# dafyddstephenson/ucla-roms

Hardware: AMD Instinct MI355X
Metric: grid-cell-updates/sec (higher is better)
Workload: dtype f64; 1 GPU; C3: basin 1024x1024x100, NONLIN+SPLIT EOS, T+S, LMD KPP/BKPP/RIMIX/NONLOCAL, dt=300s, ndtfast=60 (nfast=82); NT=2, nfast=82, parallelism=domain decomposition 1x1, halo_transport=none (single rank), fast_exchange_interval=1, exchange_order=none (single rank), s2d_window=True, comm_bootstrap=none (single rank)

## Files before the change

### include/roms_gpu.h

```cpp
#ifndef ROMS_GPU_H
#define ROMS_GPU_H

#ifdef __cplusplus
extern "C" {
#endif

#define ROMS_GPU_ABI_VERSION 18
#define ROMS_MAX_FAST 288

typedef struct roms_dims {
  int Lm, Mm, N, NT;
  int LLm, MMm;
  int np_xi, np_eta, inode, jnode;
  int iSW_corn, jSW_corn;
  int ew_periodic, ns_periodic;
  int west_exchng, east_exchng, south_exchng, north_exchng;
} roms_dims;

#define ROMS_LMD_MIXING   1
#define ROMS_LMD_KPP      2
#define ROMS_LMD_BKPP     4
#define ROMS_LMD_RIMIX    8
#define ROMS_LMD_CONVEC   16
#define ROMS_LMD_NONLOCAL 32
#define ROMS_LMD_ALL      63
#define ROMS_LMD_ICELAND  47
#define ROMS_LMD_DDMIX    64

typedef struct roms_cfg {
  int nonlin_eos;
  int salinity;
  int lmd_mixing;
  int uv_vis2, ts_dif2;
  double dt;
  int ndtfast, nfast;
  double weight[2][ROMS_MAX_FAST];
  double g, rho0, rdrg, rdrg2, Zob, gamma2;
  double Akv_bak, Akt_bak[2];
  double Tcoef, T0, Scoef, S0;
  double theta_s, theta_b, hc;
// ... 76 lines not shown

enum roms_case_id { ROMS_CASE_FILAMENT = 0, ROMS_CASE_BASIN = 1, ROMS_CASE_PIPES = 2, ROMS_CASE_RIVERS = 3 };
typedef struct roms_case {
  int case_id, LLm, MMm, N, NT;
  int salinity, nonlin_eos, lmd_mixing;
  double dt; int ndtfast;
  double sizex, sizey;
  int surf_flux;
  int obc;
  double v_sponge;
  int island;
  int curvgrid;
  int uv_adv, uv_cor;
  int bulk_frc;
  int adv_isoneutral;
} roms_case;
int roms_gpu_init_case(const roms_case *c, int device, roms_tlev *t);
int roms_gpu_init_case_comm(const roms_case *c, int np_xi, int np_eta, void *comm, int device, roms_tlev *t);

int roms_gpu_comm_unique_id(void *id128);
int roms_gpu_comm_create(const void *id128, int nranks, int rank, int device, void **comm);
int roms_gpu_comm_create_local(int group, int nranks, int rank, void **comm);
typedef int (*roms_host_allgather_fn)(void *ctx, const void *send, long nbytes, void *recv);
int roms_gpu_comm_create_host(int nranks, int rank, int device, roms_host_allgather_fn allgather, void *ctx,
                              void **comm);
int roms_gpu_comm_destroy(void *comm);
int roms_gpu_halo_transport(void);
int roms_gpu_halo_exchanges(long *per_step, int *fast_interval);
int roms_gpu_halo_overlap(void);
int roms_gpu_s2d_window(void);
#define ROMS_COLPATH_SEG 1
#define ROMS_COLPATH_GLOBAL 2
int roms_gpu_column_path(void);
int roms_gpu_horizontal_path(int out[8]);
int roms_gpu_selftest_zero_fill(long n, int chunks, long *bad);
int roms_gpu_halo_plan(int Lm, int Mm, int np_xi, int np_eta, int inode, int jnode, int ew_periodic,
                       int ns_periodic, int peer[8], long count[8], int strip[4]);
long roms_gpu_halo_map(int Lm, int Mm, int np_xi, int np_eta, int inode, int jnode, int ew_periodic,
                       int ns_periodic, int dir, int unpack, int *i, int *j, long cap);
long roms_gpu_halo_map_wide(int Lm, int Mm, int np_xi, int np_eta, int inode, int jnode, int ew_periodic,
                            int ns_periodic, int width, int dir, int unpack, int *i, int *j, long cap);

#define ROMS_FRC_SURFACE 1
#define ROMS_FRC_BRY     2
int roms_gpu_frc_record(int field_id, int slot, double rec_time, const double *data);
int roms_gpu_frc_interp(double modtime, int kinds);
int roms_gpu_frc_clock(double start_time, int on);
int roms_gpu_set_tide_data(int ntides, const double *ftide, const double *pot_re, const double *pot_im,
                           const double *ztide_re, const double *ztide_im, const double *utide_re,
                           const double *utide_im, const double *vtide_re, const double *vtide_im);
int roms_gpu_set_tides(double time);

#define ROMS_WRT_Z    1
#define ROMS_WRT_UB   2
#define ROMS_WRT_VB   4
#define ROMS_WRT_U    8
#define ROMS_WRT_V    16
#define ROMS_WRT_T    32
#define ROMS_WRT_R    64
#define ROMS_WRT_O    128
#define ROMS_WRT_AKV  256
#define ROMS_WRT_AKT  512
#define ROMS_WRT_AKS  1024
#define ROMS_WRT_HBLS 2048
#define ROMS_WRT_HBBL 4096
#define ROMS_WRT_DEFAULT 63
// ... 30 lines not shown
```

### ucla-roms_amd/csrc/k_lmd.hip

```cpp
#include <cmath>
#include <type_traits>

#include "k_common.h"

namespace roms {
namespace {

constexpr double kRicr = 0.15, kEpssfc = 0.1, kC_Ek = 258.;
constexpr double kZeta_m = -0.2, kA_m = 1.257, kC_m = 8.360, kZeta_s = -1.0, kA_s = -28.86, kC_s = 98.96;
constexpr double kEPS = 1.E-20;
constexpr double kRi0 = 0.7, kNu0m = 1.e-2, kNu0s = 1.e-2, kNuwm = 1.0e-4, kNuws = 0.1e-4, kNu0c = 0.1, kLturb = 10.;
constexpr double kPi = 3.14159265358979323;

__device__ __forceinline__ void ddmix(double t0, double t1, double s0, double s1, double zwk, double& kt,
                                      double& ks) {
  const double A0 = +0.665157E-01, A1 = +0.170907E-01, A2 = -0.203814E-03, A3 = +0.298357E-05,
               A4 = -0.255019E-07, B0 = +0.378110E-02, B1 = -0.846960E-04, C0 = -0.678662E-05,
               D0 = +0.380374E-04, D1 = -0.933746E-06, D2 = +0.791325E-08, E0 = -0.164759E-06,
               F0 = -0.251520E-11, G0 = +0.512857E-12, H0 = -0.302285E-13, Smean = 35.0;
  const double lmd_nu = 1.5e-6, lmd_Rrho0 = 1.9, lmd_nuf = 10.0e-4, lmd_fdd = 0.7, lmd_tdd1 = 0.909,
               lmd_tdd2 = 4.6, lmd_tdd3 = 0.54, lmd_sdd1 = 0.15, lmd_sdd2 = 1.85, lmd_sdd3 = 0.85, eps = 1.E-14;
  const double Tt = 0.5 * (t0 + t1);
  const double Ts = 0.5 * (s0 + s1) - Smean;
  const double Tp = -zwk;
// ... 117 lines not shown
  const Bounds& b = d.b;
  const long ij = IJ(b, i, j), n2 = b.n2;
  const int N = b.N;
  const double mu1 = 0.35, mu2 = 23.0, r1 = 0.58;
  const double attn1 = -1. / mu1, attn2 = -1. / mu2;
  double swdk1 = r1, swdk2 = 1. - swdk1;
  double* __restrict__ sw = d.f.swr_frac + ij;
  const double* __restrict__ Hz = d.f.Hz + ij;
  sw[(long)N * n2] = 1.;
  for (int k = N; k >= 1; k--) {
    const double hz = Hz[(long)(k - 1) * n2];
    const double xi1 = attn1 * hz;
    if (xi1 > -20.) swdk1 = swdk1 * exp(xi1);
    else swdk1 = 0.;
    const double xi2 = attn2 * hz;
    if (xi2 > -20.) swdk2 = swdk2 * exp(xi2);
    else swdk2 = 0.;
    sw[(long)(k - 1) * n2] = swdk1 + swdk2;
  }
}

#ifndef ROMS_KBLS_G
#define ROMS_KBLS_G 16
#endif
constexpr int kKblsG = ROMS_KBLS_G;
#ifndef ROMS_KPP_PFD
#define ROMS_KPP_PFD 1
#endif
constexpr int kKppPfd = ROMS_KPP_PFD;

#ifndef ROMS_KPP_EXT_WAVES
#define ROMS_KPP_EXT_WAVES 3
#endif
template <class C>
__global__ void __launch_bounds__(64, ROMS_KPP_EXT_WAVES) k_kpp_ext(Dev d, Range E, int tind, int nstp, KppConst kc) {
  ROMS_IJC_OR_RETURN(E)
  const Bounds& b = d.b;
  const Fields& F = d.f;
  const Params& P = d.p;
  const int N = b.N;
  const long n2 = b.n2, ij = IJ(b, i, j), sj = b.nx2;
  const double g = P.g, vonKar = P.vonKar, Ri_inv = 1. / kRicr;
  const C FCc = ColMake<C>::at(d, 0, 0, ij);
  const BufF64 FCg(d.f.colscr);
  constexpr bool kGlb = std::is_same<C, ColGlb>::value;
  auto fc_set = [&](int k, double v) {
    if constexpr (kGlb) FCg.st(v, (unsigned)ij * 8u, (unsigned)k * (unsigned)n2 * 8u);
    else FCc[k] = v;
  };
  auto fc_get = [&](int k) {
    if constexpr (kGlb) return FCg.ld((unsigned)ij * 8u, (unsigned)k * (unsigned)n2 * 8u);
    else return FCc[k];
  };
  double alpha, beta;
  const double Tt = F.t[ij + (long)(N - 1) * n2 + (long)(nstp - 1) * b.n3];
  if (P.nonlin_eos) {
    const double r01 = 6.793952E-2, r02 = -9.095290E-3, r03 = +1.001685E-4, r04 = -1.120083E-6,
                 r05 = +6.536332E-9, r10 = +0.824493, r11 = -4.08990E-3, r12 = +7.64380E-5,
                 r13 = -8.24670E-7, r14 = +5.38750E-9, rS0 = -5.72466E-3, rS1 = +1.02270E-4,
                 rS2 = -1.65460E-6, r20 = +4.8314E-4;
    const double cff = 1. / P.rho0;
    if (P.salinity) {
      const double Ts = F.t[ij + (long)(N - 1) * n2 + (long)(nstp - 1) * b.n3 + 3 * b.n3], sqrtTs = sqrt(dmax(0., Ts));
      alpha = -cff * (r01 + Tt * (2. * r02 + Tt * (3. * r03 + Tt * (4. * r04 + Tt * 5. * r05))) +
                      Ts * (r11 + Tt * (2. * r12 + Tt * (3. * r13 + Tt * 4. * r14)) + sqrtTs * (rS1 + Tt * 2. * rS2)));
      beta = cff * (r10 + Tt * (r11 + Tt * (r12 + Tt * (r13 + Tt * r14))) + 1.5 * (rS0 + Tt * (rS1 + Tt * rS2)) * sqrtTs +
                    2. * r20 * Ts);
    } else {
      alpha = -cff * (r01 + Tt * (2. * r02 + Tt * (3. * r03 + Tt * (4. * r04 + Tt * 5. * r05))));
      beta = 0.;
    }
  } else {
    alpha = fabs(P.Tcoef);
    beta = P.salinity ? fabs(P.Scoef) : 0.;
  }
  const double sr = F.srflx[ij];
  const double Bo = P.salinity ? g * (alpha * (F.stflx[ij] - sr) - beta * F.stflx[ij + n2]) : g * (alpha * (F.stflx[ij] - sr));
  const double Bosol = g * alpha * sr;
  double ustar;
  if (P.bulk_frc) {
    const double sr_ = F.sustr_r[ij], sv_ = F.svstr_r[ij];
    ustar = sqrt(sqrt(sr_ * sr_ + sv_ * sv_));
  } else {
    const double su0 = F.sustr[ij], su1 = F.sustr[ij + 1], sv0 = F.svstr[ij], sv1 = F.svstr[ij + sj];
    ustar = sqrt(sqrt(0.333333333333 * (su0 * su0 + su1 * su1 + su0 * su1 + sv0 * sv0 + sv1 * sv1 + sv0 * sv1)));
  }
  const double hbl0 = F.hbls[ij], bbl0 = F.hbbl[ij];
  const double rm = F.rmask[ij], ff = F.f[ij];
  F.lmd_Bo[ij] = Bo;
  F.lmd_Bosol[ij] = Bosol;
  F.lmd_ustar[ij] = ustar;

  const unsigned vo = (unsigned)ij * 8u, vx = vo + 8u, vy = vo + (unsigned)sj * 8u, lv = (unsigned)n2 * 8u;
  const BufF64 U(F.u + (long)(tind - 1) * b.n3), V(F.v + (long)(tind - 1) * b.n3), Hz(F.Hz), zr(F.z_r), zw(F.z_w),
      bvf(F.bvf), sw(F.swr_frac), rig(F.lmd_rig);
  const double zwN = zw.ld(vo, (unsigned)N * lv), zw0 = zw.ld(vo, 0);
  const double eh = kEpssfc * hbl0, eb = kEpssfc * bbl0;
  const double eh2 = eh * eh, eb2 = eb * eb;

  auto vtsq = [&](double zrk, double swk, double swm, double bm) {
    const double swdk_r = sqrt(swk * swm);
    const double zscale = zwN - zrk;
    const double Bfsfc = Bo + Bosol * (1. - swdk_r);
    const double ws = wscale_ws(zscale, Bfsfc, hbl0, ustar, rm, vonKar);
    return 1.8 * kc.Vtc * ws * sqrt(dmax(1.e-5, bm));
  };
  struct Lv { double u0, u1, v0, v1, hz, zr, zw, swm, bm; };
  auto ldlev = [&](int k, Lv& L) {
    const unsigned o = (unsigned)(k - 1) * lv, ow = (unsigned)k * lv;
    L.u0 = U.ld(vo, o); L.u1 = U.ld(vx, o); L.v0 = V.ld(vo, o); L.v1 = V.ld(vy, o);
    L.hz = Hz.ld(vo, o); L.zr = zr.ld(vo, o); L.zw = zw.ld(vo, ow);
    L.swm = sw.ld(vo, o); L.bm = bvf.ld(vo, o);
  };
  const unsigned oN = (unsigned)(N - 1) * lv;
  double u0p = U.ld(vo, oN), u1p = U.ld(vx, oN);
  double v0p = V.ld(vo, oN), v1p = V.ld(vy, oN);
  double hzp = Hz.ld(vo, oN), zrp = zr.ld(vo, oN);
  double swc = sw.ld(vo, oN), bc = bvf.ld(vo, oN);
  Lv cur{};
  if (N - 1 >= 1) ldlev(N - 1, cur);
  double FCk = 0.;
  fc_set(N, 0.);
  double Crp = FCk + vtsq(zrp, sw.ld(vo, (unsigned)N * lv), swc, bc);
  int kbls = Crp < 0. ? N : 0;
  double cr_k = Crp, cr_kp = 0., zr_k = zrp, zr_kp = 0.;
  for (int k = N - 1; k >= 1; k--) {
    Lv nxt = cur;
    if (k > 1) ldlev(k - 1, nxt);
    const unsigned ow = (unsigned)k * lv;
    const double u0 = cur.u0, u1 = cur.u1, v0 = cur.v0, v1 = cur.v1;
    const double hz = cur.hz, zrk = cur.zr, zwk = cur.zw, bk = bc;
    if (P.lmd_rimix) {
      const double cff = 0.5 / (zrp - zrk);
      const double dudz = cff * (u0p - u0 + u1p - u1);
      const double dvdz = cff * (v0p - v0 + v1p - v1);
      rig.st(bk / (kRi0 * dmax(dudz * dudz + dvdz * dvdz, 1.E-10)), vo, ow);
    }
    {
      const double cu = zwN - zwk, cd = zwk - zw0;
      const double cff_up = cu * cu, cff_dn = cd * cd;
      const double Kern = cff_up * cff_dn / ((cff_up + eh2) * (cff_dn + eb2));
      const double du = u0p + u1p - u0 - u1;
      const double dv = v0p + v1p - v0 - v1;
      const double hh = hz + hzp;
      FCk = FCk + Kern * (0.5 * (du * du + dv * dv) / hh - 0.5 * hh * (Ri_inv * bk + kC_Ek * ff * ff));
      fc_set(k, FCk);
    }
    const double Cr = FCk + vtsq(zrk, swc, cur.swm, cur.bm);
    if (kbls == 0 && Cr < 0.) {
      kbls = k;
      cr_k = Cr; cr_kp = Crp; zr_k = zrk; zr_kp = zrp;
    }
    Crp = Cr;
    u0p = u0; u1p = u1; v0p = v0; v1p = v1; hzp = hz; zrp = zrk;
    swc = cur.swm; bc = cur.bm;
    cur = nxt;
  }
  double fc0;
  {
    const double hz1 = hzp;
    const double z_bl = zw0 + 0.25 * hz1;
    const double cu = zwN - z_bl, cd = z_bl - zw0;
    const double cff_up = cu * cu, cff_dn = cd * cd;
    const double Kern = cff_up * cff_dn / ((cff_up + eh2) * (cff_dn + eb2));
    const double su = u0p + u1p, sv = v0p + v1p;
    fc0 = FCk + Kern * (0.5 * (su * su + sv * sv) / hz1 - 0.5 * hz1 * (Ri_inv * bvf.ld(vo, lv) + kC_Ek * ff * ff));
    fc_set(0, fc0);
  }
  double hbl;
  if (kbls > 0) {
    if (kbls == N) hbl = zwN - zr.ld(vo, oN);
    else hbl = zwN - (zr_k * cr_kp - zr_kp * cr_k) / (cr_kp - cr_k);
  } else {
    hbl = zwN - zw0;
  }
  F.lmd_hbl[ij] = hbl * rm;
  const double FC0 = fc0;
  double bbl = zwN - zw0;
  int kb = 0;
  double crk = 0., crmk = 0.;
  {
    constexpr int G = kKblsG;
    double crm = 0.;
    for (int k0 = 1; k0 <= N; k0 += G) {
      double c[G];
#pragma unroll
      for (int q = 0; q < G; q++) c[q] = fc_get(k0 + q <= N ? k0 + q : N);
#pragma unroll
      for (int q = 0; q < G; q++) {
        if (kb == 0 && k0 + q <= N) {
          const double cr = c[q] - FC0;
          if (cr > 0.) { kb = k0 + q; crk = cr; crmk = crm; }
          crm = cr;
        }
      }
      if (__all(kb != 0)) break;
    }
  }
  if (kb == 1) bbl = zr.ld(vo, 0) - zw0;
  else if (kb > 1) {
    const double zrm = zr.ld(vo + (unsigned)(kb - 2) * lv, 0u), zrk = zr.ld(vo + (unsigned)(kb - 1) * lv, 0u);
    bbl = (zrm * crk - zrk * crmk) / (crk - crmk) - zw0;
  }
  F.lmd_bbl[ij] = bbl * rm;
}

template <bool kDD, int TY = 0, int MW = 1>
__global__ void __launch_bounds__(TY > 0 ? kCX * TY : 64, MW) k_kpp_int(Dev d, Range R, EdgeClamp ec, int tind, int nstp,
                                                                   int first, KppConst kc) {
  constexpr bool STG = TY > 0;
  constexpr int TYB = STG ? TY : 1, WW = kCX + 2, WN = WW * (TYB + 2), NTH = kCX * TYB, WQ = (WN + NTH - 1) / NTH;
  const uint3 bI = xcd_tile();
  const int ti0 = tile_i0(R.i0);
  int i = ti0 + (int)(bI.x * kCX + threadIdx.x);
  int j = R.j0 + (int)(bI.y * TYB + threadIdx.y);
  const bool act = i >= R.i0 && i <= R.i1 && j <= R.j1;
  if (!STG && !act) return;
  if (!act) { i = i < R.i0 ? R.i0 : (i < R.i1 ? i : R.i1); j = j < R.j1 ? j : R.j1; }
  __shared__ double sW[STG ? 2 : 1][STG ? WN : 1];
  const int tid = threadIdx.x + kCX * threadIdx.y;
  const int wi0 = ti0 + (int)bI.x * kCX - 1, wj0 = R.j0 + (int)bI.y * TYB - 1;
  const Bounds& b = d.b;
  const Fields& F = d.f;
  const Params& P = d.p;
  const int N = b.N;
  const long n2 = b.n2, ij = IJ(b, i, j), sj = b.nx2;
  const double vonKar = P.vonKar, Zob = P.Zob;
  const double akv = P.Akv_bak, akt = P.Akt_bak[0], aks = P.Akt_bak[b.nTS - 1];
  const double rm = F.rmask[ij];
  const SmoothMasks m = smooth_masks(b, F, i, j);
  double w[3][3];
  load3x3(b, ec, F.lmd_hbl, i, j, w);
  double hbl = smooth_point(w, m) * rm;
  load3x3(b, ec, F.lmd_bbl, i, j, w);
  double bbl = smooth_point(w, m) * rm;
  if (!first) {
    hbl = 0.5 * (hbl + F.hbls[ij]);
    bbl = 0.5 * (bbl + F.hbbl[ij]);
  }
  const unsigned vo = (unsigned)ij * 8u, lv = (unsigned)n2 * 8u;
  const BufF64 zw(F.z_w), sw(F.swr_frac);
  const double zwN = zw.ld(vo, (unsigned)N * lv), zw0 = zw.ld(vo, 0);
  int kbls = N;
  {
    constexpr int G = kKblsG;
    for (int k0 = N - 1; k0 >= 1; k0 -= G) {
      double z[G];
#pragma unroll
      for (int q = 0; q < G; q++) z[q] = zw.ld(vo, (unsigned)(k0 - q >= 1 ? k0 - q : 1) * lv);
#pragma unroll
      for (int q = 0; q < G; q++)
        if (k0 - q >= 1 && z[q] > zwN - hbl) kbls = k0 - q;
    }
  }
  const double Bo = F.lmd_Bo[ij], Bosol = F.lmd_Bosol[ij], ustar = F.lmd_ustar[ij];
  double Bfsfc;
  {
    const double z_bl = zwN - hbl;
    const unsigned ok = vo + (unsigned)kbls * lv, om = vo + (unsigned)(kbls - 1) * lv;
    const double swm = sw.ld(om, 0u), swk = sw.ld(ok, 0u);
    const double zwk = zw.ld(ok, 0u), zwm = zw.ld(om, 0u);
    if (swm > 0.)
      Bfsfc = Bo + Bosol * (1. - swm * swk * (zwk - zwm) / (swk * (zwk - z_bl) + swm * (z_bl - zwm)));
    else
      Bfsfc = Bo + Bosol;
  }
  double wmb;
  {
    const long o = (long)(nstp - 1) * b.n3 + ij;
    const double u0 = F.u[o], u1 = F.u[o + 1], v0 = F.v[o], v1 = F.v[o + sj];
    wmb = vonKar * vonKar * sqrt(0.333333333333 * (u0 * u0 + u1 * u1 + u0 * u1 + v0 * v0 + v1 * v1 + v0 * v1)) /
          log(1. + 0.5 * F.Hz[ij] / Zob);
  }
  const double wsb = wmb;

  const double* __restrict__ rig = F.lmd_rig;
  const BufF64 Rg(F.lmd_rig);
  unsigned wo[STG ? WQ : 1];
  if constexpr (STG) {
#pragma unroll
    for (int m = 0; m < WQ; m++) {
      const int q = tid + m * NTH;
      wo[m] = q < WN ? (unsigned)ec.at(b, wi0 + q % WW, wj0 + q / WW) * 8u : kBufOff;
    }
  }
// ... 141 lines not shown
  if (E) { F.hbls[ij + 1] = hbl; F.hbbl[ij + 1] = bbl; }
  if (S) { F.hbls[ij - sj] = hbl; F.hbbl[ij - sj] = bbl; }
  if (Nn) { F.hbls[ij + sj] = hbl; F.hbbl[ij + sj] = bbl; }
  if (W && S) { F.hbls[ij - 1 - sj] = hbl; F.hbbl[ij - 1 - sj] = bbl; }
  if (W && Nn) { F.hbls[ij - 1 + sj] = hbl; F.hbbl[ij - 1 + sj] = bbl; }
  if (E && S) { F.hbls[ij + 1 - sj] = hbl; F.hbbl[ij + 1 - sj] = bbl; }
  if (E && Nn) { F.hbls[ij + 1 + sj] = hbl; F.hbbl[ij + 1 + sj] = bbl; }
}

}

void launch_swr_frac(const Dev& d, hipStream_t s) {
  const Bounds& b = d.b;
  const Range R{b.istr, b.iend, b.jstr, b.jend};
  hipLaunchKernelGGL(k_swr_frac, grid_of(R), dim3(kBX, kBY), 0, s, d, R);
  ExchList L{};
  L.p[0] = d.f.swr_frac; L.nlev[0] = b.N + 1; L.n = 1;
  launch_exchange_list(d, s, L);
}

void launch_lmd_vmix(const Dev& d, hipStream_t s, const Tlev& t, int tind) {
  const Bounds& b = d.b;
  Range E;
  E.i0 = (b.ew_periodic || !b.west_edge) ? b.istr - 1 : b.istr;
  E.i1 = (b.ew_periodic || !b.east_edge) ? b.iend + 1 : b.iend;
  E.j0 = (b.ns_periodic || !b.south_edge) ? b.jstr - 1 : b.jstr;
  E.j1 = (b.ns_periodic || !b.north_edge) ? b.jend + 1 : b.jend;
  const Range R{b.istr, b.iend, b.jstr, b.jend};
  const double vonKar = d.p.vonKar, Cstar = 10., c_s = kC_s, epssfc = kEpssfc, Cv = 1.8, betaT = -0.2;
  KppConst kc;
  kc.Cg = Cstar * vonKar * std::pow(c_s * vonKar * epssfc, 1. / 3.);
  kc.Vtc = Cv * std::sqrt(-betaT / (c_s * epssfc)) / (kRicr * (vonKar * vonKar));
  const int first = t.iic == t.forw_start;
  if (d.f.colscr)
    hipLaunchKernelGGL(k_kpp_ext<ColGlb>, gridc_of(E), dim3(kCX), 0, s, d, E, tind, t.nstp, kc);
  else
    hipLaunchKernelGGL(k_kpp_ext<ColLds>, gridc_of(E), dim3(kCX), col_lds_bytes(1, b.N), s, d, E, tind, t.nstp, kc);
  if (d.p.kpp_ty && d.p.lmd_rimix) {
    const int ty = d.p.lmd_ddmix ? 4 : (d.p.kpp_ty == 8 || d.p.kpp_ty == 2) ? d.p.kpp_ty : 4;
    dim3 g = gridc_of(R);
    g.y = (g.y + ty - 1) / ty;
    const EdgeClamp ec = edge_clamp(b);
    if (d.p.lmd_ddmix)
      hipLaunchKernelGGL((k_kpp_int<true, 4>), g, dim3(kCX, 4), 0, s, d, R, ec, tind, t.nstp, first, kc);
    else if (d.p.kpp_ty == 2)
      hipLaunchKernelGGL((k_kpp_int<false, 2>), g, dim3(kCX, 2), 0, s, d, R, ec, tind, t.nstp, first, kc);
    else if (d.p.kpp_ty == 8)
      hipLaunchKernelGGL((k_kpp_int<false, 8>), g, dim3(kCX, 8), 0, s, d, R, ec, tind, t.nstp, first, kc);
    else if (d.p.kpp_ty == 43)
      hipLaunchKernelGGL((k_kpp_int<false, 4, 3>), g, dim3(kCX, 4), 0, s, d, R, ec, tind, t.nstp, first, kc);
    else
      hipLaunchKernelGGL((k_kpp_int<false, 4>), g, dim3(kCX, 4), 0, s, d, R, ec, tind, t.nstp, first, kc);
  } else if (d.p.lmd_ddmix) {
    hipLaunchKernelGGL(k_kpp_int<true>, gridc_of(R), dim3(kCX), 0, s, d, R, edge_clamp(b), tind, t.nstp, first, kc);
  } else {
    hipLaunchKernelGGL(k_kpp_int<false>, gridc_of(R), dim3(kCX), 0, s, d, R, edge_clamp(b), tind, t.nstp, first, kc);
  }
  ExchList L{};
  L.p[0] = d.f.Akv; L.nlev[0] = b.N + 1;
  L.p[1] = d.f.hbls; L.nlev[1] = 1;
  L.p[2] = d.f.hbbl; L.nlev[2] = 1;
  L.p[3] = d.f.Akt; L.nlev[3] = (b.N + 1) * b.nTS;
  L.n = 4;
  launch_exchange_list(d, s, L);
}

}
// ... 1 lines not shown
```

### ucla-roms_amd/csrc/roms_dev.h

```cpp
#pragma once
#include <hip/hip_runtime.h>
#include <cstddef>
#include <cstdint>

namespace roms {

constexpr int kMaxFast = 288;
constexpr int kRowAlign = 16;
constexpr int kAlignOff = 14;

struct Bounds {
  int Lm, Mm, N, NT, nTS, nx2;
  long n2, n3, n3w;
  int gx;
  int istr, iend, jstr, jend;
  int istrU, istrR, iendR, jstrV, jstrR, jendR;
  int istrE, iendE, jstrE, jendE;
  int west_edge, east_edge, south_edge, north_edge;
  int ew_periodic, ns_periodic;
  int west_exch, east_exch, south_exch, north_exch;
};

struct Params {
  int nonlin_eos, salinity, lmd, uv_vis2, ts_dif2;
// ... 14 lines not shown
  int s2d_fold;
  int hoist;
  int chain_dirz;
  int prs_fuse_uv;
  int h_ty;
  int h_jc;
  int prs_ty;
  int ld16;
  int prs_buf;
  int prs_strip;
  int t_strip;
  int visc_stg;
  int t3dmix_stg;
  int kpp_ty;
  int tile_grp;
  int uv1_lds;
  int omega_seg;
  int omega_cw;
  int omega_ord;
  int omega_par;
  int p_in_rho;
  int omega_hb;
  int preuv_lds;
  int seg_jrows;
  int t_chunk;
  int seg_buf;
  int seg_vtile;
  int s2d_k;
  int uv2e_nc, uv2e_nf;
  int npip;
  int nriv, nrivf;
  int curvgrid;
  int obc;
  double ubind;
  double dt, dtfast, g, rho0, vonKar, qp2, gamma2, hc;
  double rdrg, Zob, Tcoef, T0, Scoef, S0;
  double Akv_bak, Akt_bak[2];
};

struct Fields {
  double *h, *hinv, *f, *fomn, *pm, *pn, *dm_r, *dn_r, *dm_u, *dn_u, *dm_v, *dn_v, *dm_p, *dn_p,
      *pmon_u, *pnom_v, *rmask, *pmask, *umask, *vmask;
  double *dndx, *dmde;
  double* ptide;
  double *uwnd, *vwnd, *tair, *qair, *prate, *swrad, *lwrad, *sustr_r, *svstr_r;
  double *Cs_w, *Cs_r;
  double *zeta, *ubar, *vbar, *u, *v, *t;
  double *FlxU, *FlxV, *We, *Wi, *Hz, *Hz_u, *Hz_v, *z_r, *z_w;
  double *rufrc, *rvfrc, *rhoA, *rhoS, *r_D, *Zt_avg1, *DU_avg1, *DV_avg1, *DU_avg2, *DV_avg2,
      *DU_avg_bak, *DV_avg_bak;
  double *rho, *rho1, *qp1, *bvf, *Akv, *Akt, *visc2_r, *visc2_p, *diff2;
  double *hbls, *hbbl, *ghat, *swr_frac;
  double *sustr, *svstr, *stflx, *srflx, *swflx;
  double *ru, *rv, *P, *rhos;
  double *c0, *c1, *c2, *c3;
  double *s0, *s1, *s2, *s3, *s4, *s5, *s6, *s7, *s8, *s9;
  double *lmd_rig, *lmd_hbl, *lmd_bbl, *lmd_Bo, *lmd_Bosol, *lmd_ustar;
  int* pipe_idx;
  double *pipe_flx, *pipe_prf, *pipe_trc;
  double *riv_uflx, *riv_vflx, *riv_vol, *riv_trc;
  int* riv_face;
  int *uv2e_couple, *uv2e_flux;
  double *bzeta[4], *bubar[4], *bvbar[4], *bu[4], *bv[4], *bt[4];
  double* ub[4];
  double* colscr;
  double *dRdx, *dRde, *idRz, *diff3u, *diff3v, *Akz;
// ... 211 lines not shown
void setup_omega_seg();
bool omega_takes_seg(const Dev& d, int width);
int s2d_edge_mode(const Dev& d);
int s2d_edge_modes_taken(bool reset = false);
bool prsgrd_takes_strips(const Dev& d, bool with_uv, int& jA, int& jB, int& nstrip);
double pre_step3d_dtau(const Dev& d, const Tlev& t);
void launch_rho_eos(const Dev& d, hipStream_t s, const Tlev& t, int tidx);
void launch_prsgrd(const Dev& d, hipStream_t s, const Tlev& t, int uv_up = -1, bool p_ready = false);
bool launch_tracer_strip(const Dev& d, hipStream_t s, const Range& R, int mode, bool up, bool hb_done, int nnew,
                         int nrhs, double dtau, double cf_stp, double cf_bak, int nstp, int& jA, int& jB);
bool p_in_rho(const Dev& d);
void launch_prsgrd_P(const Dev& d, hipStream_t s);
bool prsgrd_can_fuse_uv(const Dev& d);
struct Side {
  hipStream_t s2;
  hipEvent_t efork, ejoin;
};
void launch_pre_step3d(const Dev& d, hipStream_t s, const Tlev& t, bool uv_done = false, bool hb_done = false,
                       const Side* side = nullptr);
void launch_step3d_uv1(const Dev& d, hipStream_t s, const Tlev& t, bool uv_done = false);
void launch_visc3d(const Dev& d, hipStream_t s, const Tlev& t);
void launch_step2d(const Dev& d, hipStream_t s, const Tlev& t, const double* w1, const double* w2);
void launch_step3d_uv2(const Dev& d, hipStream_t s, const Tlev& t);
void launch_step3d_t(const Dev& d, hipStream_t s, const Tlev& t, bool exchange = true);
void launch_t3dmix(const Dev& d, hipStream_t s, const Tlev& t);
void launch_u3dbc(const Dev& d, hipStream_t s, const Tlev& t);
void launch_river_s2d(const Dev& d, hipStream_t s, int knew);
void launch_bulk_flux(const Dev& d, hipStream_t s, int nrhs);
void launch_river_uv(const Dev& d, hipStream_t s, int nnew, int pred);
void launch_v3dbc(const Dev& d, hipStream_t s, const Tlev& t);
void launch_t3dbc(const Dev& d, hipStream_t s, const Tlev& t, int itrc);
void launch_diag(const Dev& d, hipStream_t s, const Tlev& t, double* out);
void launch_swr_frac(const Dev& d, hipStream_t s);
void launch_lmd_vmix(const Dev& d, hipStream_t s, const Tlev& t, int tind);
void launch_iso_slopes(const Dev& d, hipStream_t s);
void launch_iso_diff3(const Dev& d, hipStream_t s, const Tlev& t, int iu0, int iu1, int iv0, int iv1, int j0, int j1);
void launch_iso_exch_diff3(const Dev& d, hipStream_t s);
void launch_iso_tracer(const Dev& d, hipStream_t s, const Tlev& t, int itrc);

}
```

### ucla-roms_amd/csrc/roms_shim.cpp

```cpp
#include <hip/hip_runtime.h>

#include <algorithm>
#include <cmath>
#include <cstdlib>
#include <cstdio>
#include <cstring>
#include <map>
#include <string>
#include <vector>

#include "../../include/roms_gpu.h"
#include "halo.h"
#include "host_init.h"
#include "roms_dev.h"
#include "shim_state.h"

using namespace roms;

namespace {

struct FieldDesc {
  double* d = nullptr;
  long count = 0;
  long hcount = 0;
// ... 750 lines not shown
    P.preuv_lds = !(e && e[0] == '0');
  }
  {
    const char* e = getenv("ROMS_GPU_HTY");
    P.h_ty = (e && atoi(e) == 8) ? 8 : 4;
  }
  {
    const char* e = getenv("ROMS_GPU_HJC");
    P.h_jc = 0;
    if (e && atoi(e) >= 0) P.h_jc = atoi(e) / 4 * 4;
  }
  {
    const char* e = getenv("ROMS_GPU_PRS_TY");
    P.prs_ty = (e && atoi(e) == 8) ? 8 : 4;
  }
  {
    const char* e = getenv("ROMS_GPU_LD16");
    P.ld16 = g.off != 0 && e && e[0] == '1';
  }
  {
    const char* e = getenv("ROMS_GPU_VISC_STG");
    P.visc_stg = !(e && e[0] == '0');
  }
  {
    const char* e = getenv("ROMS_GPU_T3DMIX_STG");
    P.t3dmix_stg = !(e && e[0] == '0');
  }
  {
    const char* e = getenv("ROMS_GPU_KPP_TY");
    P.kpp_ty = 4;
    if (e && (atoi(e) == 0 || atoi(e) == 2 || atoi(e) == 8 || atoi(e) == 43)) P.kpp_ty = atoi(e);
  }
  {
    const char* e = getenv("ROMS_GPU_HOIST");
    P.hoist = !(e && e[0] == '0');
  }
  {
    const char* e = getenv("ROMS_GPU_PRS_BUF");
    P.prs_buf = !(e && e[0] == '0');
  }
  {
    const char* e = getenv("ROMS_GPU_PRS_STRIP");
    P.prs_strip = !(e && e[0] == '0');
  }
  {
    const char* e = getenv("ROMS_GPU_T_STRIP");
    P.t_strip = e && e[0] == '1';
  }
  {
    const char* e = getenv("ROMS_GPU_TCHUNK");
    P.t_chunk = e ? atoi(e) : 0;
    if (P.t_chunk < 0) P.t_chunk = 0;
  }
  {
    const char* e = getenv("ROMS_GPU_SEG_BUF");
    P.seg_buf = e ? atoi(e) : 679;
  }
  {
    const char* e = getenv("ROMS_GPU_SEG_VTILE");
    P.seg_vtile = !(e && e[0] == '0');
  }
  P.seg_jrows = kSegJMax < 2 ? kSegJMax : 2;
  {
    const char* e = getenv("ROMS_GPU_SEG_JROWS");
    if (e && atoi(e) >= 1 && atoi(e) <= kSegJMax) P.seg_jrows = atoi(e);
  }
// ... 221 lines not shown
    return post_launch();             \
  }
ROUTINE(roms_gpu_set_huv, (launch_set_huv(g.d, g.s, T), g.hzuv_valid = true))
ROUTINE(roms_gpu_omega, launch_omega(g.d, g.s, T))
ROUTINE(roms_gpu_prsgrd, launch_prsgrd(g.d, g.s, T))
ROUTINE(roms_gpu_pre_step3d, launch_pre_step3d(g.d, g.s, T))
ROUTINE(roms_gpu_set_huv1, launch_set_huv1(g.d, g.s, T))
ROUTINE(roms_gpu_step3d_uv1, launch_step3d_uv1(g.d, g.s, T))
ROUTINE(roms_gpu_visc3d, launch_visc3d(g.d, g.s, T))
ROUTINE(roms_gpu_step3d_uv2, launch_step3d_uv2(g.d, g.s, T))
ROUTINE(roms_gpu_step3d_t, launch_step3d_t(g.d, g.s, T))
ROUTINE(roms_gpu_t3dmix, launch_t3dmix(g.d, g.s, T))
ROUTINE(roms_gpu_set_depth, launch_set_depth(g.d, g.s, T))
#undef ROUTINE

int roms_gpu_halo_transport(void) {
  REQUIRE_INIT_NOJOIN();
  return g.d.halo ? halo_transport(g.halo) : 0;
}

int roms_gpu_halo_overlap(void) {
  REQUIRE_INIT_NOJOIN();
  return g.d.halo && g.halo.xoverlap > 0 ? 1 : 0;
}

int roms_gpu_s2d_window(void) {
  REQUIRE_INIT_NOJOIN();
  return g.d.w2.base ? 1 : 0;
}

int roms_gpu_column_path(void) {
  REQUIRE_INIT_NOJOIN();
  return (g.d.p.colseg ? ROMS_COLPATH_SEG : 0) | (g.d.f.colscr ? ROMS_COLPATH_GLOBAL : 0);
}

int roms_gpu_horizontal_path(int out[8]) {
  REQUIRE_INIT_NOJOIN();
  if (!out) { g.err = "roms_gpu_horizontal_path: null argument"; return -1; }
  const Dev& d = g.d;
  int jA = 0, jB = -1, nstrip = 0;
  const bool strips = prsgrd_takes_strips(d, prsgrd_can_fuse_uv(d), jA, jB, nstrip);
  out[0] = s2d_edge_mode(d);
  out[1] = strips ? 1 : 0;
  out[2] = strips ? nstrip : 0;
  out[3] = strips ? jA : 0;
  out[4] = strips ? jB : -1;
  out[5] = omega_takes_seg(d, d.b.iend - d.b.istr + 1) ? 1 : 0;
  out[6] = s2d_edge_modes_taken();
  out[7] = 0;
  return 0;
}

int roms_gpu_halo_exchanges(long* per_step, int* fast_interval) {
  REQUIRE_INIT_NOJOIN();
  if (per_step) *per_step = g.step_exch;
  if (fast_interval) *fast_interval = g.d.p.s2d_k;
  return 0;
}

int roms_gpu_step2d(const roms_tlev* t) {
  REQUIRE_INIT_NOJOIN();
  REQUIRE_HALO_OK();
  const Tlev T = to_tlev(t);
  launch_step2d(g.d, g.s, T, g.w1, g.w2);
  return post_launch();
}
// ... 549 lines not shown
```

### ucla-roms_amd/romsgpu/__init__.py

```python
import ctypes
import os

import numpy as np

_HERE = os.path.dirname(os.path.abspath(__file__))
_PKG = os.path.dirname(_HERE)
LIB_PATH = os.environ.get("ROMS_GPU_LIB") or os.path.join(_PKG, "libromsgpu.so")
MAX_FAST = 288

FIELDS = ["h", "hinv", "f", "fomn", "pm", "pn", "dm_r", "dn_r", "dm_u", "dn_u", "dm_v", "dn_v", "dm_p", "dn_p",
          "pmon_u", "pnom_v", "rmask", "pmask", "umask", "vmask", "Cs_w", "Cs_r",
          "zeta", "ubar", "vbar", "u", "v", "t", "FlxU", "FlxV", "We", "Wi", "Hz", "Hz_u", "Hz_v", "z_r", "z_w",
          "rufrc", "rvfrc", "rhoA", "rhoS", "r_D", "Zt_avg1", "DU_avg1", "DV_avg1", "DU_avg2", "DV_avg2",
          "DU_avg_bak", "DV_avg_bak", "rho", "rho1", "qp1", "bvf", "Akv", "Akt", "visc2_r", "visc2_p", "diff2",
          "hbls", "hbbl", "ghat", "swr_frac", "sustr", "svstr", "stflx", "srflx", "swflx", "ru", "rv"] + \
         ["%s_%s" % (v, e) for v in ("zeta", "ubar", "vbar", "u", "v", "t") for e in ("west", "east", "south", "north")] + \
         ["dndx", "dmde", "ptide", "uwnd", "vwnd", "tair", "qair", "prate", "swrad", "lwrad", "sustr_r", "svstr_r"]
FIELD_ID = {n: i for i, n in enumerate(FIELDS)}
CASE_FILAMENT, CASE_BASIN, CASE_PIPES, CASE_RIVERS = 0, 1, 2, 3
LMD_MIXING, LMD_KPP, LMD_BKPP, LMD_RIMIX, LMD_CONVEC, LMD_NONLOCAL = 1, 2, 4, 8, 16, 32
LMD_DDMIX = 64
LMD_ALL = 63
LMD_ICELAND = 47

# ... 421 lines not shown
    def step3d_t(self): self._r("step3d_t")
    def t3dmix(self): self._r("t3dmix")
    def set_depth(self): self._r("set_depth")
    def swr_frac(self): self._r("swr_frac")
    def init_sequence(self): self._r("init_sequence")

    def step(self, n=1):
        for _ in range(n):
            self._r("step")

    def time_routine(self, routine, nsteps):
        ms = ctypes.c_double()
        n = ctypes.c_long()
        self._chk(self.L.roms_gpu_time_routine(ROUTINES.index(routine), nsteps, ctypes.byref(self.t), ctypes.byref(ms),
                                               ctypes.byref(n)), "time_routine")
        return ms.value, n.value

    def selftest_zero_fill(self, n, chunks=1):
        nz = ctypes.c_long()
        self._chk(self.L.roms_gpu_selftest_zero_fill(ctypes.c_long(n), ctypes.c_int(chunks), ctypes.byref(nz)),
                  "selftest_zero_fill")
        return nz.value

    def halo_transport(self):
        r = self.L.roms_gpu_halo_transport()
        return {1: "ipc", 0: "rccl", -1: "ipc-timeout"}.get(r, "error")

    def halo_overlap(self):
        return bool(self.L.roms_gpu_halo_overlap())

    def s2d_window(self):
        return bool(self.L.roms_gpu_s2d_window())

    def column_path(self):
        r = self.L.roms_gpu_column_path()
        self._chk(min(r, 0), "column_path")
        return bool(r & 1), bool(r & 2)

    def horizontal_path(self):
        out = (ctypes.c_int * 8)()
        self._chk(self.L.roms_gpu_horizontal_path(out), "horizontal_path")
        return {"edges": out[0], "strips": (out[2], out[3], out[4]) if out[1] else None, "omega_seg": bool(out[5])}

    def fast_step_edge_modes(self):
        out = (ctypes.c_int * 8)()
        self._chk(self.L.roms_gpu_horizontal_path(out), "horizontal_path")
        return {m for m in range(3) if out[6] >> m & 1}

    def halo_exchanges(self):
        n, k = ctypes.c_long(), ctypes.c_int()
        self._chk(self.L.roms_gpu_halo_exchanges(ctypes.byref(n), ctypes.byref(k)), "halo_exchanges")
        return n.value, k.value

    def diag(self):
        out = (ctypes.c_double * 4)()
        self._chk(self.L.roms_gpu_diag(ctypes.byref(self.t), out), "diag")
        return list(out)

    def time(self, dt):
        return dt * (self.t.iic - self.t.ntstart + 1) + getattr(self, "start_time", 0.0)

    def wrt_rst(self, path, rec, total_rec, time):
        self._chk(self.L.roms_gpu_wrt_rst(path.encode(), rec, total_rec, time, ctypes.byref(self.t)), "wrt_rst")

    def wrt_his(self, path, rec, total_rec, time, mask=WRT_DEFAULT):
        self._chk(self.L.roms_gpu_wrt_his(path.encode(), rec, total_rec, time, ctypes.byref(self.t), mask), "wrt_his")
# ... 34 lines not shown
```

Baseline: 2.240 billion cell-updates/s.

## Trim KPP column work with wave-level early exits and bounded LDS storage

In the KPP extension kernel, the surface boundary-layer search stops computing Cr and loading shortwave fractions once every lane in the wavefront has found kbls. The bulk-Richardson integral FC is now kept in LDS only for the bottom 16 levels; a rare fallback recomputes the upper levels from global memory when the bottom-layer search fails within that window. The kbls search in the later kernel also breaks early once all lanes are below the boundary layer. The intent is to cut redundant loads and arithmetic and to shrink LDS per block for better occupancy, at the cost of more code paths and a slow fallback.

Measured after the change: 2.281 billion cell-updates/s (median of 6 runs). 1.02x the previous value.

```diff
diff --git a/include/roms_gpu.h b/include/roms_gpu.h
--- a/include/roms_gpu.h
+++ b/include/roms_gpu.h
@@ -5,7 +5,7 @@
 extern "C" {
 #endif
 
-#define ROMS_GPU_ABI_VERSION 18
+#define ROMS_GPU_ABI_VERSION 19
 #define ROMS_MAX_FAST 288
 
 typedef struct roms_dims {
@@ -148,6 +148,7 @@
 #define ROMS_COLPATH_SEG 1
 #define ROMS_COLPATH_GLOBAL 2
 int roms_gpu_column_path(void);
+int roms_gpu_kpp_lean(void);
 int roms_gpu_horizontal_path(int out[8]);
 int roms_gpu_selftest_zero_fill(long n, int chunks, long *bad);
 int roms_gpu_halo_plan(int Lm, int Mm, int np_xi, int np_eta, int inode, int jnode, int ew_periodic,
diff --git a/ucla-roms_amd/csrc/k_lmd.hip b/ucla-roms_amd/csrc/k_lmd.hip
--- a/ucla-roms_amd/csrc/k_lmd.hip
+++ b/ucla-roms_amd/csrc/k_lmd.hip
@@ -173,7 +173,7 @@
 #ifndef ROMS_KPP_EXT_WAVES
 #define ROMS_KPP_EXT_WAVES 3
 #endif
-template <class C>
+template <class C, bool KEEP = false>
 __global__ void __launch_bounds__(64, ROMS_KPP_EXT_WAVES) k_kpp_ext(Dev d, Range E, int tind, int nstp, KppConst kc) {
   ROMS_IJC_OR_RETURN(E)
   const Bounds& b = d.b;
@@ -185,9 +185,11 @@
   const C FCc = ColMake<C>::at(d, 0, 0, ij);
   const BufF64 FCg(d.f.colscr);
   constexpr bool kGlb = std::is_same<C, ColGlb>::value;
+  static_assert(!KEEP || std::is_same<C, ColLds>::value, "KEEP: the LDS slot");
+  const int keep = KEEP ? (P.kpp_fckeep < N ? P.kpp_fckeep : N) : N;
   auto fc_set = [&](int k, double v) {
     if constexpr (kGlb) FCg.st(v, (unsigned)ij * 8u, (unsigned)k * (unsigned)n2 * 8u);
-    else FCc[k] = v;
+    else if (!KEEP || k <= keep) FCc[k] = v;
   };
   auto fc_get = [&](int k) {
     if constexpr (kGlb) return FCg.ld((unsigned)ij * 8u, (unsigned)k * (unsigned)n2 * 8u);
@@ -247,11 +249,21 @@
     return 1.8 * kc.Vtc * ws * sqrt(dmax(1.e-5, bm));
   };
   struct Lv { double u0, u1, v0, v1, hz, zr, zw, swm, bm; };
-  auto ldlev = [&](int k, Lv& L) {
+  auto ldlev = [&](int k, Lv& L, bool need_sw) {
     const unsigned o = (unsigned)(k - 1) * lv, ow = (unsigned)k * lv;
     L.u0 = U.ld(vo, o); L.u1 = U.ld(vx, o); L.v0 = V.ld(vo, o); L.v1 = V.ld(vy, o);
     L.hz = Hz.ld(vo, o); L.zr = zr.ld(vo, o); L.zw = zw.ld(vo, ow);
-    L.swm = sw.ld(vo, o); L.bm = bvf.ld(vo, o);
+    L.swm = sw.ld(need_sw ? vo : kBufOff, o); L.bm = bvf.ld(vo, o);
+  };
+  auto fc_term = [&](double u0p, double u1p, double v0p, double v1p, double hzp, double u0, double u1, double v0,
+                     double v1, double hz, double zwk, double bk) {
+    const double cu = zwN - zwk, cd = zwk - zw0;
+    const double cff_up = cu * cu, cff_dn = cd * cd;
+    const double Kern = cff_up * cff_dn / ((cff_up + eh2) * (cff_dn + eb2));
+    const double du = u0p + u1p - u0 - u1;
+    const double dv = v0p + v1p - v0 - v1;
+    const double hh = hz + hzp;
+    return Kern * (0.5 * (du * du + dv * dv) / hh - 0.5 * hh * (Ri_inv * bk + kC_Ek * ff * ff));
   };
   const unsigned oN = (unsigned)(N - 1) * lv;
   double u0p = U.ld(vo, oN), u1p = U.ld(vx, oN);
@@ -259,15 +271,17 @@
   double hzp = Hz.ld(vo, oN), zrp = zr.ld(vo, oN);
   double swc = sw.ld(vo, oN), bc = bvf.ld(vo, oN);
   Lv cur{};
-  if (N - 1 >= 1) ldlev(N - 1, cur);
+  if (N - 1 >= 1) ldlev(N - 1, cur, true);
   double FCk = 0.;
   fc_set(N, 0.);
   double Crp = FCk + vtsq(zrp, sw.ld(vo, (unsigned)N * lv), swc, bc);
   int kbls = Crp < 0. ? N : 0;
   double cr_k = Crp, cr_kp = 0., zr_k = zrp, zr_kp = 0.;
+  const bool skipv = (P.kpp_lean & 1) != 0;
+  bool vdone = skipv && __all(kbls != 0);
   for (int k = N - 1; k >= 1; k--) {
     Lv nxt = cur;
-    if (k > 1) ldlev(k - 1, nxt);
+    if (k > 1) ldlev(k - 1, nxt, !vdone);
     const unsigned ow = (unsigned)k * lv;
     const double u0 = cur.u0, u1 = cur.u1, v0 = cur.v0, v1 = cur.v1;
     const double hz = cur.hz, zrk = cur.zr, zwk = cur.zw, bk = bc;
@@ -277,24 +291,20 @@
       const double dvdz = cff * (v0p - v0 + v1p - v1);
       rig.st(bk / (kRi0 * dmax(dudz * dudz + dvdz * dvdz, 1.E-10)), vo, ow);
     }
-    {
-      const double cu = zwN - zwk, cd = zwk - zw0;
-      const double cff_up = cu * cu, cff_dn = cd * cd;
-      const double Kern = cff_up * cff_dn / ((cff_up + eh2) * (cff_dn + eb2));
-      const double du = u0p + u1p - u0 - u1;
-      const double dv = v0p + v1p - v0 - v1;
-      const double hh = hz + hzp;
-      FCk = FCk + Kern * (0.5 * (du * du + dv * dv) / hh - 0.5 * hh * (Ri_inv * bk + kC_Ek * ff * ff));
-      fc_set(k, FCk);
-    }
-    const double Cr = FCk + vtsq(zrk, swc, cur.swm, cur.bm);
-    if (kbls == 0 && Cr < 0.) {
-      kbls = k;
-      cr_k = Cr; cr_kp = Crp; zr_k = zrk; zr_kp = zrp;
-    }
-    Crp = Cr;
+    FCk = FCk + fc_term(u0p, u1p, v0p, v1p, hzp, u0, u1, v0, v1, hz, zwk, bk);
+    fc_set(k, FCk);
+    if (!vdone) {
+      const double Cr = FCk + vtsq(zrk, swc, cur.swm, cur.bm);
+      if (kbls == 0 && Cr < 0.) {
+        kbls = k;
+        cr_k = Cr; cr_kp = Crp; zr_k = zrk; zr_kp = zrp;
+      }
+      Crp = Cr;
+      swc = cur.swm;
+      vdone = skipv && __all(kbls != 0);
+    }
     u0p = u0; u1p = u1; v0p = v0; v1p = v1; hzp = hz; zrp = zrk;
-    swc = cur.swm; bc = cur.bm;
+    bc = cur.bm;
     cur = nxt;
   }
   double fc0;
@@ -323,19 +333,39 @@
   {
     constexpr int G = kKblsG;
     double crm = 0.;
-    for (int k0 = 1; k0 <= N; k0 += G) {
+    for (int k0 = 1; k0 <= keep; k0 += G) {
       double c[G];
 #pragma unroll
-      for (int q = 0; q < G; q++) c[q] = fc_get(k0 + q <= N ? k0 + q : N);
+      for (int q = 0; q < G; q++) c[q] = fc_get(k0 + q <= keep ? k0 + q : keep);
 #pragma unroll
       for (int q = 0; q < G; q++) {
-        if (kb == 0 && k0 + q <= N) {
+        if (kb == 0 && k0 + q <= keep) {
           const double cr = c[q] - FC0;
           if (cr > 0.) { kb = k0 + q; crk = cr; crmk = crm; }
           crm = cr;
         }
       }
       if (__all(kb != 0)) break;
+    }
+  }
+  if constexpr (KEEP) {
+    if (keep < N && !__all(kb != 0)) {
+      double u0p = U.ld(vo, oN), u1p = U.ld(vx, oN), v0p = V.ld(vo, oN), v1p = V.ld(vy, oN), hzp = Hz.ld(vo, oN);
+      double FCf = 0.;
+      double crp = 0. - FC0;
+      int kf = 0;
+      double crkf = 0., crmf = 0.;
+      for (int k = N - 1; k > keep; k--) {
+        const unsigned o = (unsigned)(k - 1) * lv, ow = (unsigned)k * lv;
+        const double u0 = U.ld(vo, o), u1 = U.ld(vx, o), v0 = V.ld(vo, o), v1 = V.ld(vy, o), hz = Hz.ld(vo, o);
+        FCf = FCf + fc_term(u0p, u1p, v0p, v1p, hzp, u0, u1, v0, v1, hz, zw.ld(vo, ow), bvf.ld(vo, ow));
+        const double cr = FCf - FC0;
+        if (crp > 0.) { kf = k + 1; crkf = crp; crmf = cr; }
+        crp = cr;
+        u0p = u0; u1p = u1; v0p = v0; v1p = v1; hzp = hz;
+      }
+      if (crp > 0.) { kf = keep + 1; crkf = crp; crmf = fc_get(keep) - FC0; }
+      if (kb == 0 && kf != 0) { kb = kf; crk = crkf; crmk = crmf; }
     }
   }
   if (kb == 1) bbl = zr.ld(vo, 0) - zw0;
@@ -385,13 +415,19 @@
   int kbls = N;
   {
     constexpr int G = kKblsG;
+    const bool early = (P.kpp_lean & 4) != 0;
+    bool below = false;
     for (int k0 = N - 1; k0 >= 1; k0 -= G) {
       double z[G];
 #pragma unroll
       for (int q = 0; q < G; q++) z[q] = zw.ld(vo, (unsigned)(k0 - q >= 1 ? k0 - q : 1) * lv);
 #pragma unroll
       for (int q = 0; q < G; q++)
-        if (k0 - q >= 1 && z[q] > zwN - hbl) kbls = k0 - q;
+        if (k0 - q >= 1) {
+          if (z[q] > zwN - hbl) kbls = k0 - q;
+          else below = true;
+        }
+      if (early && __all(below)) break;
     }
   }
   const double Bo = F.lmd_Bo[ij], Bosol = F.lmd_Bosol[ij], ustar = F.lmd_ustar[ij];
@@ -599,7 +635,10 @@
   kc.Cg = Cstar * vonKar * std::pow(c_s * vonKar * epssfc, 1. / 3.);
   kc.Vtc = Cv * std::sqrt(-betaT / (c_s * epssfc)) / (kRicr * (vonKar * vonKar));
   const int first = t.iic == t.forw_start;
-  if (d.f.colscr)
+  if (d.p.kpp_lean & 2)
+    hipLaunchKernelGGL((k_kpp_ext<ColLds, true>), gridc_of(E), dim3(kCX),
+                       col_lds_bytes(1, d.p.kpp_fckeep < b.N ? d.p.kpp_fckeep : b.N), s, d, E, tind, t.nstp, kc);
+  else if (d.f.colscr)
     hipLaunchKernelGGL(k_kpp_ext<ColGlb>, gridc_of(E), dim3(kCX), 0, s, d, E, tind, t.nstp, kc);
   else
     hipLaunchKernelGGL(k_kpp_ext<ColLds>, gridc_of(E), dim3(kCX), col_lds_bytes(1, b.N), s, d, E, tind, t.nstp, kc);
diff --git a/ucla-roms_amd/csrc/roms_dev.h b/ucla-roms_amd/csrc/roms_dev.h
--- a/ucla-roms_amd/csrc/roms_dev.h
+++ b/ucla-roms_amd/csrc/roms_dev.h
@@ -70,6 +70,8 @@
   int nriv, nrivf;
   int curvgrid;
   int obc;
+  short kpp_lean;
+  short kpp_fckeep;
   double ubind;
   double dt, dtfast, g, rho0, vonKar, qp2, gamma2, hc;
   double rdrg, Zob, Tcoef, T0, Scoef, S0;
@@ -347,6 +349,7 @@
 void launch_t3dbc(const Dev& d, hipStream_t s, const Tlev& t, int itrc);
 void launch_diag(const Dev& d, hipStream_t s, const Tlev& t, double* out);
 void launch_swr_frac(const Dev& d, hipStream_t s);
+constexpr int kKppFcKeepMax = 16;
 void launch_lmd_vmix(const Dev& d, hipStream_t s, const Tlev& t, int tind);
 void launch_iso_slopes(const Dev& d, hipStream_t s);
 void launch_iso_diff3(const Dev& d, hipStream_t s, const Tlev& t, int iu0, int iu1, int iv0, int iv1, int j0, int j1);
diff --git a/ucla-roms_amd/csrc/roms_shim.cpp b/ucla-roms_amd/csrc/roms_shim.cpp
--- a/ucla-roms_amd/csrc/roms_shim.cpp
+++ b/ucla-roms_amd/csrc/roms_shim.cpp
@@ -806,6 +806,14 @@
     if (e && (atoi(e) == 0 || atoi(e) == 2 || atoi(e) == 8 || atoi(e) == 43)) P.kpp_ty = atoi(e);
   }
   {
+    const char* e = getenv("ROMS_GPU_KPP_LEAN");
+    P.kpp_lean = 7;
+    if (e && e[0] >= '0' && e[0] <= '7' && e[1] == 0) P.kpp_lean = e[0] - '0';
+    const char* k = getenv("ROMS_GPU_KPP_FCKEEP");
+    P.kpp_fckeep = kKppFcKeepMax;
+    if (k && atoi(k) >= 1 && atoi(k) <= kKppFcKeepMax) P.kpp_fckeep = atoi(k);
+  }
+  {
     const char* e = getenv("ROMS_GPU_HOIST");
     P.hoist = !(e && e[0] == '0');
   }
@@ -1093,6 +1101,11 @@
 int roms_gpu_column_path(void) {
   REQUIRE_INIT_NOJOIN();
   return (g.d.p.colseg ? ROMS_COLPATH_SEG : 0) | (g.d.f.colscr ? ROMS_COLPATH_GLOBAL : 0);
+}
+
+int roms_gpu_kpp_lean(void) {
+  REQUIRE_INIT_NOJOIN();
+  return g.d.p.kpp_lean + 256 * g.d.p.kpp_fckeep;
 }
 
 int roms_gpu_horizontal_path(int out[8]) {
diff --git a/ucla-roms_amd/romsgpu/__init__.py b/ucla-roms_amd/romsgpu/__init__.py
--- a/ucla-roms_amd/romsgpu/__init__.py
+++ b/ucla-roms_amd/romsgpu/__init__.py
@@ -477,6 +477,11 @@
     def s2d_window(self):
         return bool(self.L.roms_gpu_s2d_window())
 
+    def kpp_lean(self):
+        r = self.L.roms_gpu_kpp_lean()
+        self._chk(min(r, 0), "kpp_lean")
+        return r % 256, r // 256
+
     def column_path(self):
         r = self.L.roms_gpu_column_path()
         self._chk(min(r, 0), "column_path")
```
